# hzi-bifo/Quasimodo

Hardware: AMD Instinct MI355X
Metric: variant TP/FP classifications/sec across all caller x sample VCFs (higher is better)
Workload: dtype int32; 1 GPU; BASELINE configs[2]: 1000 VCFs x 1 M SNPs/GPU, 5 Mb ref, 100000 truth keys, 256-bin ROC, sorted; vcfs_per_gpu=1000, records_per_vcf=1000000, parallelism=vcf-shard x1, collective=none

## Files before the change

quasimodo_amd/csrc/qmvt_kernels.hip:

```cpp
#include <type_traits>
#include <hip/hip_runtime.h>
#include <stdint.h>
#include <stdlib.h>
#include <string.h>

#include "qmvt_dev.h"

namespace qm {

template <typename T> __device__ __forceinline__ T ntl(const T* p) {
  return __builtin_nontemporal_load(p);
}
template <typename T> __device__ __forceinline__ void nts(T* p, T v) {
  __builtin_nontemporal_store(v, p);
}
__device__ __forceinline__ int lane_id() { return (int)(threadIdx.x & 63); }
__device__ __forceinline__ uint64_t ballot64(bool p) { return __ballot(p); }
__device__ __forceinline__ int popc64(uint64_t x) { return __popcll(x); }

__device__ __forceinline__ int qual_bin(float q, int n_bins) {
  if (!(q >= 0.0f)) return -1;
  if (q >= (float)n_bins) return n_bins - 1;
  return (int)q;
}

__device__ __forceinline__ bool is_snp(int r, int a) { return ((uint32_t)r < 4u) & ((uint32_t)a < 4u); }
__device__ __forceinline__ uint32_t pack_key(int p, int r, int a) {
  return ((uint32_t)p << 4) | ((uint32_t)r << 2) | (uint32_t)a;
}

__device__ __forceinline__ int lds_lower_bound(const uint32_t* __restrict__ k, int m, int top, uint32_t key) {
  int pos = 0;
  for (int step = top; step > 0; step >>= 1) {
    int idx = pos + step;
    int rd = idx <= m ? idx - 1 : m - 1;
    uint32_t v = k[rd];
    if (idx <= m && v < key) pos = idx;
  }
  return pos;
}


constexpr uint32_t I_BIN1 = 0x1ffu;
constexpr uint32_t I_PASS = 1u << 9;
constexpr uint32_t I_IDDOT = 1u << 10;
constexpr uint32_t I_NOKEY = 1u << 11;
constexpr uint32_t I_LIVE = 1u << 12;
constexpr uint32_t I_BADPOS = 1u << 13;
constexpr uint32_t I_KEPT = 1u << 16;
constexpr uint32_t I_IDDOT4 = 1u << 20;
constexpr uint32_t I_TPLINE = 1u << 24;

__device__ __forceinline__ void pack_record_nib(int p, bool alive, uint32_t nib, float q, uint32_t fl, int nb, uint32_t& key, uint32_t& inf) {
  const bool okpos = (uint32_t)p < (uint32_t)QM_POS_LIMIT_DEV;
  const bool live = okpos && alive;
  key = ((uint32_t)p << 4) | (live ? nib : 0u);
  inf = (live ? (uint32_t)(qual_bin(q, nb) + 1) : 0u) | ((fl & 7u) << 9) | (live ? I_LIVE : 0u) | (okpos ? 0u : I_BADPOS) |
        ((live && (fl & QMF_PASS)) ? I_KEPT : 0u) | ((fl & QMF_IDDOT) ? I_IDDOT4 : 0u) | ((live && (fl & QMF_TPLINE)) ? I_TPLINE : 0u);
}
__device__ __forceinline__ void pack_record(int p, uint32_t d, float q, uint32_t fl, int nb, uint32_t& key, uint32_t& inf) {
  d &= 0xffu;
  pack_record_nib(p, d < 16u, d, q, fl, nb, key, inf);
}
__device__ __forceinline__ void pack_record_ext(int p, int r, int a, float q, uint32_t fl, int nb, uint32_t& key, uint32_t& inf) {
  pack_record_nib(p, allele_valid(r) && allele_valid(a), allele_nib(r, a), q, fl, nb, key, inf);
}

__host__ __device__ inline uint32_t flag_info(uint32_t f) {
  return ((f & 7u) << 9) | I_LIVE | ((f & QMF_PASS) ? I_KEPT : 0u) | ((f & QMF_IDDOT) ? I_IDDOT4 : 0u) | ((f & QMF_TPLINE) ? I_TPLINE : 0u);
}

__device__ __forceinline__ void pack_record_fast(int p, uint32_t d, float q, uint32_t f4x4 , float nbm1f,
                                                 const uint32_t* flut, uint32_t& key, uint32_t& inf) {
  const bool live = ((uint32_t)p | (d << 24)) < (uint32_t)QM_POS_LIMIT_DEV;
  key = ((uint32_t)p << 4) | (live ? d : 0u);
  const float c = fminf(fmaxf(q, -1.0f), nbm1f);
  const uint32_t b1 = (uint32_t)((int)floorf(c) + 1);
  const uint32_t g = *reinterpret_cast<const uint32_t*>(reinterpret_cast<const char*>(flut) + f4x4);
  inf = live ? (b1 | g) : 0u;
}

__device__ __forceinline__ void pack_record_fast_ext(int p, int r, int a, float q, uint32_t f4x4, float nbm1f, const uint32_t* flut,
                                                     uint32_t& key, uint32_t& inf) {
  const uint32_t ur = (uint32_t)r, ua = (uint32_t)a;
  constexpr uint32_t VALID_BY_CLZ = 0xC000001Eu;
  const uint32_t ok = (VALID_BY_CLZ >> __builtin_clz(ur | 1u)) & (VALID_BY_CLZ >> __builtin_clz(ua | 1u)) & 1u;
  const bool live = ((uint32_t)p >> 28) < ok;
  const uint32_t nib = ((ur << 2) ^ ua ^ ((ur ^ ua) >> 4)) & 15u;
  key = ((uint32_t)p << 4) | (live ? nib : 0u);
  const float c = fminf(fmaxf(q, -1.0f), nbm1f);
  const uint32_t b1 = (uint32_t)((int)floorf(c) + 1);
  const uint32_t g = *reinterpret_cast<const uint32_t*>(reinterpret_cast<const char*>(flut) + f4x4);
  inf = live ? (b1 | g) : 0u;
}

struct Cols {
  const int32_t* pos;
  const int32_t* ref;
  const int32_t* alt;
  const float* qual;
  const uint8_t* flags;
  const uint8_t* anib;
  const uint32_t* pkey;
  const uint32_t* pinf;
};

template <bool PACKED> struct Raw4;
template <> struct Raw4<false> { int4 p, r, a; float4 q; uint32_t f, d; };
template <> struct Raw4<true> { uint4 k, i; int4 r, a; };

template <bool EXT>
__device__ __forceinline__ void load_raw(const Cols& C, int idx, Raw4<false>& R) {
  typedef int v4i __attribute__((ext_vector_type(4)));
  typedef float v4f __attribute__((ext_vector_type(4)));
  const v4i vp = __builtin_nontemporal_load(reinterpret_cast<const v4i*>(C.pos + idx));
  if (EXT) {
    const v4i vr = __builtin_nontemporal_load(reinterpret_cast<const v4i*>(C.ref + idx));
    const v4i va = __builtin_nontemporal_load(reinterpret_cast<const v4i*>(C.alt + idx));
    R.r = make_int4(vr.x, vr.y, vr.z, vr.w);
    R.a = make_int4(va.x, va.y, va.z, va.w);
  } else {
    R.d = __builtin_nontemporal_load(reinterpret_cast<const uint32_t*>(C.anib + idx));
  }
  const v4f vq = __builtin_nontemporal_load(reinterpret_cast<const v4f*>(C.qual + idx));
  R.p = make_int4(vp.x, vp.y, vp.z, vp.w);
  R.q = make_float4(vq.x, vq.y, vq.z, vq.w);
  R.f = __builtin_nontemporal_load(reinterpret_cast<const uint32_t*>(C.flags + idx));
}
template <bool EXT>
__device__ __forceinline__ void load_raw(const Cols& C, int idx, Raw4<true>& R) {
  typedef unsigned v4u __attribute__((ext_vector_type(4)));
  const v4u vk = __builtin_nontemporal_load(reinterpret_cast<const v4u*>(C.pkey + idx));
  const v4u vi = __builtin_nontemporal_load(reinterpret_cast<const v4u*>(C.pinf + idx));
  R.k = make_uint4(vk.x, vk.y, vk.z, vk.w);
  R.i = make_uint4(vi.x, vi.y, vi.z, vi.w);
  if (EXT) {
    R.r = *reinterpret_cast<const int4*>(C.ref + idx);
    R.a = *reinterpret_cast<const int4*>(C.alt + idx);
  }
}

struct In4 {
  uint32_t key[4], inf[4];
  int32_t r[4], a[4];
  uint32_t posor;
};

template <bool EXT>
__device__ __forceinline__ void unpack_raw(const Raw4<false>& R, int nb, In4& X, const uint32_t* flut) {
  const float nbm1f = (float)(nb - 1);
  if (!EXT) {
    pack_record_fast(R.p.x, R.d & 0xffu, R.q.x, (R.f << 2) & 0x3cu, nbm1f, flut, X.key[0], X.inf[0]);
    pack_record_fast(R.p.y, (R.d >> 8) & 0xffu, R.q.y, (R.f >> 6) & 0x3cu, nbm1f, flut, X.key[1], X.inf[1]);
    pack_record_fast(R.p.z, (R.d >> 16) & 0xffu, R.q.z, (R.f >> 14) & 0x3cu, nbm1f, flut, X.key[2], X.inf[2]);
    pack_record_fast(R.p.w, R.d >> 24, R.q.w, (R.f >> 22) & 0x3cu, nbm1f, flut, X.key[3], X.inf[3]);
  } else {
    pack_record_fast_ext(R.p.x, R.r.x, R.a.x, R.q.x, (R.f << 2) & 0x3cu, nbm1f, flut, X.key[0], X.inf[0]);
    pack_record_fast_ext(R.p.y, R.r.y, R.a.y, R.q.y, (R.f >> 6) & 0x3cu, nbm1f, flut, X.key[1], X.inf[1]);
    pack_record_fast_ext(R.p.z, R.r.z, R.a.z, R.q.z, (R.f >> 14) & 0x3cu, nbm1f, flut, X.key[2], X.inf[2]);
    pack_record_fast_ext(R.p.w, R.r.w, R.a.w, R.q.w, (R.f >> 22) & 0x3cu, nbm1f, flut, X.key[3], X.inf[3]);
    X.r[0] = R.r.x; X.r[1] = R.r.y; X.r[2] = R.r.z; X.r[3] = R.r.w;
    X.a[0] = R.a.x; X.a[1] = R.a.y; X.a[2] = R.a.z; X.a[3] = R.a.w;
  }
  X.posor = (uint32_t)R.p.x | (uint32_t)R.p.y | (uint32_t)R.p.z | (uint32_t)R.p.w;
}
template <bool EXT>
__device__ __forceinline__ void unpack_raw(const Raw4<true>& R, int, In4& X, const uint32_t*) {
  X.posor = 0u;
  if (EXT) {
    X.r[0] = R.r.x; X.r[1] = R.r.y; X.r[2] = R.r.z; X.r[3] = R.r.w;
    X.a[0] = R.a.x; X.a[1] = R.a.y; X.a[2] = R.a.z; X.a[3] = R.a.w;
  }
  X.key[0] = R.k.x; X.key[1] = R.k.y; X.key[2] = R.k.z; X.key[3] = R.k.w;
  X.inf[0] = R.i.x; X.inf[1] = R.i.y; X.inf[2] = R.i.z; X.inf[3] = R.i.w;
}

typedef const __attribute__((address_space(4))) int32_t* ci32p;
typedef const __attribute__((address_space(4))) uint32_t* cu32p;
__device__ __forceinline__ int uload(const int32_t* p, int i) { return ((ci32p)(uintptr_t)p)[i]; }
__device__ __forceinline__ uint32_t uload(const uint32_t* p, int i) { return ((cu32p)(uintptr_t)p)[i]; }
template <bool PACKED> __device__ __forceinline__ int rec_pos_uniform(const Cols& C, int i) {
  if (PACKED) return (int)(uload(C.pkey, i) >> 4);
  return uload(C.pos, i);
}

template <bool PACKED> __device__ __forceinline__ int rec_pos(const Cols& C, int i) {
  if (PACKED) return (int)(C.pkey[i] >> 4);
  return C.pos[i];
}
template <bool PACKED, bool EXT = false>
__device__ __forceinline__ void rec_packed(const Cols& C, int i, int nb, uint32_t& key, uint32_t& inf) {
  if (PACKED) { key = C.pkey[i]; inf = C.pinf[i]; return; }
  if (EXT) pack_record_ext(C.pos[i], C.ref[i], C.alt[i], C.qual[i], C.flags[i], nb, key, inf);
  else pack_record(C.pos[i], C.anib[i], C.qual[i], C.flags[i], nb, key, inf);
}

typedef const __attribute__((address_space(1))) uint32_t* gu32p;
typedef const __attribute__((address_space(1))) int32_t* gi32p;
struct TruthG {
  gu32p keys;
  gi32p tidx;
  gi32p ref, alt;
  int32_t shift, nb;
};
template <bool EXT>
__device__ __forceinline__ TruthG truth_global(const TruthDev& t) {
  TruthG g;
  if (EXT) {
    g.keys = (gu32p)t.xkeys; g.tidx = (gi32p)t.xtidx; g.ref = (gi32p)t.xref; g.alt = (gi32p)t.xalt; g.shift = t.xshift; g.nb = t.xnb;
  } else {
    g.keys = (gu32p)t.keys; g.tidx = (gi32p)t.tidx; g.ref = nullptr; g.alt = nullptr; g.shift = t.shift; g.nb = t.nb;
  }
  return g;
}

constexpr int H_PACK = 1;
constexpr int L_HTP = 0;
constexpr int L_HFP = 130;
constexpr int L_HU = 260;
constexpr int L_KEYS = 388;
__device__ __forceinline__ void hist_add(uint32_t* lds, int table, uint32_t slot) {
  if (H_PACK) atomicAdd(&lds[table + (slot >> 1)], 1u << (16u * (slot & 1u)));
  else atomicAdd(&lds[table + slot], 1u);
}
__device__ __forceinline__ uint32_t hist_get(const uint32_t* lds, int table, uint32_t slot) {
  return H_PACK ? (lds[table + (slot >> 1)] >> (16u * (slot & 1u))) & 0xffffu : lds[table + slot];
}
constexpr int L_SMAX = L_KEYS + K1_SLICE;
constexpr int L_SRF = L_SMAX + K1_SLICE;
constexpr int L_RKEY = (L_SRF + K1_SLICE / 32 + 3) & ~3;
constexpr int L_RINF = L_RKEY + 288;
constexpr int L_HITS = L_RINF + 128;
constexpr int L_FLUT = L_HITS + 8;
constexpr int L_TCNT = L_FLUT + 16;
#ifndef QM_MASK_TILES
#define QM_MASK_TILES 8
#endif
#ifndef QM_MASK_TILES_X
#define QM_MASK_TILES_X 4
#endif

template <bool EXT> __device__ __forceinline__ constexpr int mask_tiles() { return EXT ? QM_MASK_TILES_X : QM_MASK_TILES; }
constexpr int L_MASK = (L_TCNT + 2 * SPAN_TILES + 3) & ~3;
constexpr int L_TOTAL = L_MASK + 64 * QM_MASK_TILES;
constexpr int L_XRREF = L_MASK + 64 * QM_MASK_TILES_X;
constexpr int L_XRALT = L_XRREF + 256;
constexpr int L_TOTAL_X = L_XRALT + 256;
constexpr int SLICE_CAP_X = K1_SLICE / 2;
template <bool EXT> __device__ __forceinline__ constexpr int slice_cap() { return EXT ? SLICE_CAP_X : K1_SLICE; }
static_assert(L_XRREF % 4 == 0, "b128 LDS stores need natural alignment");
static_assert(L_RKEY % 4 == 0 && L_RINF % 2 == 0, "b128 / b64 LDS stores need natural alignment");
static_assert(K1_ROUNDS == 4, "a tile is 32 + 32 mask words");
static_assert(SPAN_TILES % QM_MASK_TILES == 0 && SPAN_TILES % QM_MASK_TILES_X == 0 && (32 * QM_MASK_TILES) % 8 == 0, "mask batches tile the span");
static_assert(K1_ROUNDS >= 3 && K1_SLICE % 64 == 0, "the next tile's slice is fetched over rounds 0..2 of the current one");

__device__ __forceinline__ int rk(int i) { return L_RKEY + i + ((i >> 5) << 2); }

struct Slice {
  int keys, smax, srf;
  int ref, alt;
  int m;
};

__device__ __forceinline__ void slice_select(Slice& S) {
  S.keys = L_KEYS;
  S.smax = L_SMAX;
  S.srf = L_SRF;
  S.ref = L_KEYS + SLICE_CAP_X;
  S.alt = L_SMAX + SLICE_CAP_X;
}

template <bool EXT>
__device__ __forceinline__ void stage_slice(uint32_t* lds, const TruthG& tr, int c0, const Slice& S, int lane) {
  for (int j = lane; j < S.m; j += 64) {
    lds[S.keys + j] = tr.keys[c0 + j];
    lds[S.smax + j] = 0;
    if (EXT) { lds[S.ref + j] = (uint32_t)tr.ref[c0 + j]; lds[S.alt + j] = (uint32_t)tr.alt[c0 + j]; }
  }
  if (lane < K1_SLICE / 32) lds[S.srf + lane] = 0;
}

__device__ __forceinline__ void slice_range(const TruthG& tr, int a, int b, int& lo, int& hi) {
  uint32_t ba = (uint32_t)a >> tr.shift;
  uint32_t bb = ((uint32_t)b >> tr.shift) + 1u;
  const uint32_t lim = (uint32_t)tr.nb + 1u;
  ba = ba < lim ? ba : lim;
  bb = bb < lim ? bb : lim;
  lo = uload((const int32_t*)(uintptr_t)tr.tidx, (int)ba);
  hi = uload((const int32_t*)(uintptr_t)tr.tidx, (int)bb);
  if (hi < lo) hi = lo;
}

struct SegBounds {
  int a, b;
  int prevp, nextp;
};

template <bool PACKED> __device__ __forceinline__ SegBounds seg_bounds(const Cols& C, int sb, int se, int vn) {
  SegBounds t;
  t.a = rec_pos_uniform<PACKED>(C, sb);
  t.b = rec_pos_uniform<PACKED>(C, se - 1);
  t.prevp = (sb > 0) ? rec_pos_uniform<PACKED>(C, sb - 1) : INT32_MIN;
  t.nextp = (se < vn) ? rec_pos_uniform<PACKED>(C, se) : INT32_MIN;
  return t;
}

template <bool EXT>
__device__ __forceinline__ void stage_round(uint32_t* lds, In4& X, int i0, int te, int lane) {
  if (i0 - lane * 4 + 256 > te) {
#pragma unroll
    for (int k = 0; k < 4; ++k)
      if (i0 + k >= te) { X.key[k] = 0xffffffffu; X.inf[k] = 0u; }
  }
  uint4 kv;
  kv.x = X.key[0]; kv.y = X.key[1]; kv.z = X.key[2]; kv.w = X.key[3];
  uint2 iv;
  iv.x = (X.inf[0] & 0xffffu) | (X.inf[1] << 16); iv.y = (X.inf[2] & 0xffffu) | (X.inf[3] << 16);
  *reinterpret_cast<uint4*>(&lds[rk(lane * 4)]) = kv;
  *reinterpret_cast<uint2*>(&lds[L_RINF + lane * 2]) = iv;
  if (EXT) {
    uint4 rv, av;
    rv.x = (uint32_t)X.r[0]; rv.y = (uint32_t)X.r[1]; rv.z = (uint32_t)X.r[2]; rv.w = (uint32_t)X.r[3];
    av.x = (uint32_t)X.a[0]; av.y = (uint32_t)X.a[1]; av.z = (uint32_t)X.a[2]; av.w = (uint32_t)X.a[3];
    *reinterpret_cast<uint4*>(&lds[L_XRREF + lane * 4]) = rv;
    *reinterpret_cast<uint4*>(&lds[L_XRALT + lane * 4]) = av;
  }
  if (lane < 8) lds[L_HITS + lane] = 0;
}

template <bool EXT>
__device__ __forceinline__ void join_round(uint32_t* lds, const Slice& S, int nrec, int own_a, int lane) {
  if (S.m <= 0 || nrec <= 0) return;
  const uint32_t first_pos = lds[rk(0)] >> 4;
  const uint32_t last_pos = lds[rk(nrec - 1)] >> 4;
  int rlo = 0, rhi = 0;
  for (int base = 0; base < S.m; base += 64) {
    const int j = base + lane;
    const uint32_t kp = j < S.m ? lds[S.keys + j] >> 4 : 0xffffffffu;
    rlo += popc64(ballot64(kp < first_pos));
    rhi += popc64(ballot64(kp <= last_pos));
  }
  for (int base = rlo; base < rhi; base += 64) {
    const int j = base + lane;
    if (j < rhi) {
      const uint32_t kkey = lds[S.keys + j];
      const uint32_t kpos = kkey >> 4;
      const uint32_t kfloor = kkey & ~15u;
      int pp = 0;
#pragma unroll
      for (int st = 144; st >= 36; st >>= 1)
        if (lds[L_RKEY + pp + st - 5] < kfloor) pp += st;
#pragma unroll
      for (int st = 16; st > 0; st >>= 1)
        if (lds[L_RKEY + pp + st - 1] < kfloor) pp += st;
      int s = pp - 4 * ((pp * 1821) >> 16);
      if (s < 256 && lds[L_RKEY + pp] < kfloor) s += 1;
      uint32_t mx = 0, rf = 0;
      for (; s < nrec; ++s) {
        const uint32_t rkey = lds[rk(s)];
        if ((rkey & ~15u) != kfloor) break;
        if (rkey != kkey) continue;
        if (EXT) {
          if (lds[L_XRREF + s] != lds[S.ref + j] || lds[L_XRALT + s] != lds[S.alt + j]) continue;
        }
        const uint32_t inf = (lds[L_RINF + (s >> 1)] >> (16 * (s & 1))) & 0xffffu;
        if ((inf & (I_LIVE | I_NOKEY)) != I_LIVE) continue;
        atomicOr(&lds[L_HITS + (s >> 5)], 1u << (s & 31));
        if ((int)kpos != own_a) {
          const uint32_t b1 = inf & I_BIN1;
          if ((inf & I_IDDOT) && b1 > mx) mx = b1;
          rf |= (inf & I_PASS) ? 1u : 0u;
        }
      }
      if (mx) atomicMax(&lds[S.smax + j], mx);
      if (rf) atomicOr(&lds[S.srf + (j >> 5)], 1u << (j & 31));
    }
  }
}

__device__ __forceinline__ int slice_lower_bound(const uint32_t* lds, const Slice& S, uint32_t key) {
  int lo = 0, n = S.m;
  while (n > 0) {
    const int h = n >> 1;
    if (lds[S.keys + lo + h] < key) { lo += h + 1; n -= h + 1; } else n = h;
  }
  return lo;
}

template <bool PACKED, bool EXT>
__device__ __forceinline__ void continue_run(const Cols& C, uint32_t* lds, const Slice& S, int se, int vn, int bpos, int nb, int lane) {
  for (int base = se; base < vn; base += 64) {
    const int i = base + lane;
    bool cont = false;
    if (i < vn) {
      cont = (rec_pos<PACKED>(C, i) == bpos);
      if (cont && S.m > 0) {
        uint32_t key, inf;
        rec_packed<PACKED, EXT>(C, i, nb, key, inf);
        if ((inf & (I_LIVE | I_NOKEY)) == I_LIVE) {
          int j = slice_lower_bound(lds, S, key);
          if (EXT) {
            const uint32_t rr = (uint32_t)C.ref[i], aa = (uint32_t)C.alt[i];
            while (j < S.m && lds[S.keys + j] == key && (lds[S.ref + j] != rr || lds[S.alt + j] != aa)) ++j;
          }
          if (j < S.m && lds[S.keys + j] == key) {
            if (inf & I_IDDOT) atomicMax(&lds[S.smax + j], inf & I_BIN1);
            if (inf & I_PASS) atomicOr(&lds[S.srf + (j >> 5)], 1u << (j & 31));
          }
        }
      }
    }
    if (ballot64(cont) != ~0ull) break;
  }
}

__device__ __forceinline__ uint32_t flush_slice(uint32_t* lds, const Slice& S, int lane) {
  uint32_t tpr = 0;
  for (int j = lane; j < S.m; j += 64) {
    const uint32_t mx = lds[S.smax + j];
    if (mx) hist_add(lds, L_HU, mx - 1u);
    tpr += (lds[S.srf + (j >> 5)] >> (j & 31)) & 1u;
  }
  return tpr;
}

constexpr int X_WALK_LIMIT = 1 << 14;
template <bool PACKED, bool EXT>
__device__ __forceinline__ uint32_t repeated_key(const Cols& C, int i, uint32_t key, uint32_t nokey, int nb, int32_t r, int32_t a,
                                                 uint32_t& bad) {
  for (int j = i - 1; j >= 0; --j) {
    if (EXT && i - j > X_WALK_LIMIT) { bad |= 4u; break; }
    if (rec_pos<PACKED>(C, j) != (int)(key >> 4)) break;
    uint32_t kj, ij;
    rec_packed<PACKED, EXT>(C, j, nb, kj, ij);
    if (kj == key && (ij & (I_LIVE | I_PASS)) == (I_LIVE | I_PASS) && (ij & I_NOKEY) == nokey) {
      if (!EXT || (C.ref[j] == r && C.alt[j] == a)) return 1u;
    }
  }
  return 0u;
}

struct Acc {
  uint32_t bad;
  uint32_t fpr;
  uint32_t n_pass, n_tp;
  uint32_t top_tp, top_fp;
  uint32_t posor;
};

__device__ __forceinline__ uint32_t or_reduce8(uint32_t v) {
  v |= (uint32_t)__builtin_amdgcn_update_dpp(0, (int)v, 0x111, 0xf, 0xf, false);
  v |= (uint32_t)__builtin_amdgcn_update_dpp(0, (int)v, 0x112, 0xf, 0xf, false);
  v |= (uint32_t)__builtin_amdgcn_update_dpp(0, (int)v, 0x114, 0xf, 0xf, false);
  return v;
}

template <bool PACKED, bool EXT>
__device__ __forceinline__ void classify_round(uint32_t* lds, const Cols& C, const In4& X, int rbase, int te, int prev_last, int nb,
                                               int mslot, Acc& A, int lane) {
  const uint32_t hit = (lds[L_HITS + (lane >> 3)] >> (4 * (lane & 7))) & 15u;
  uint32_t nib = 0, anyinf = 0;
#pragma unroll
  for (int k = 0; k < 4; ++k) {
    nib |= (X.inf[k] >> 16) << k;
    anyinf |= X.inf[k];
  }
  const uint32_t pass = nib & 15u, iddot = (nib >> 4) & 15u, tpline = (nib >> 8) & 15u;
  A.bad |= ((anyinf & I_BADPOS) | (X.posor >> 28)) ? 2u : 0u;
  A.posor |= X.posor;
  const uint32_t tpkey = (hit & iddot) | tpline;
  const uint32_t tp = pass & tpkey;
  const uint32_t fpkey = pass & ~hit;
  A.n_pass += (uint32_t)__popc(pass);
  A.n_tp += (uint32_t)__popc(tp);
  A.fpr += (uint32_t)__popc(fpkey);
  {
    const uint32_t sh = 4u * (uint32_t)(lane & 7);
    const uint32_t wp = or_reduce8(pass << sh);
    const uint32_t wt = or_reduce8(tp << sh);
    if ((lane & 7) == 7) {
      lds[L_MASK + mslot + (lane >> 3)] = wp;
      lds[L_MASK + 32 * mask_tiles<EXT>() + mslot + (lane >> 3)] = wt;
    }
  }
  int pp = __shfl_up((int)(X.key[3] >> 4), 1);
  if (lane == 0) pp = prev_last;
  const int i0 = rbase + lane * 4;
  uint32_t cand = 0;
#pragma unroll
  for (int k = 0; k < 4; ++k) {
    const int p = (int)(X.key[k] >> 4);
    A.bad |= (p < pp) ? 1u : 0u;
    cand |= ((p == pp) ? 1u : 0u) << k;
    {
      const uint32_t b1 = X.inf[k] & I_BIN1;
      const uint32_t notp = ((~tpkey) >> k) & 1u;
      const bool top = b1 == (uint32_t)nb;
      const uint64_t mtop = ballot64(top);
      if (mtop) {
        const uint32_t ntp = (uint32_t)popc64(ballot64(top && !notp));
        A.top_tp += ntp;
        A.top_fp += (uint32_t)popc64(mtop) - ntp;
      }
      if (!top) hist_add(lds, notp ? L_HFP : L_HTP, b1);
    }
    pp = p;
  }
  cand &= fpkey;
  if (cand) {
#pragma unroll
    for (int k = 0; k < 4; ++k)
      if ((cand >> k) & 1u) {
        const int32_t rr = EXT ? (int32_t)lds[L_XRREF + lane * 4 + k] : 0, aa = EXT ? (int32_t)lds[L_XRALT + lane * 4 + k] : 0;
        A.fpr -= repeated_key<PACKED, EXT>(C, i0 + k, X.key[k], X.inf[k] & I_NOKEY, nb, rr, aa, A.bad);
      }
  }
}

__device__ __forceinline__ uint32_t wave_sum(uint32_t v) {
#define QM_DPP_ADD(ctrl, rmask) v += (uint32_t)__builtin_amdgcn_update_dpp(0, (int)v, ctrl, rmask, 0xf, false)
  QM_DPP_ADD(0xb1, 0xf);
  QM_DPP_ADD(0x4e, 0xf);
  QM_DPP_ADD(0x141, 0xf);
  QM_DPP_ADD(0x140, 0xf);
  QM_DPP_ADD(0x142, 0xa);
  QM_DPP_ADD(0x143, 0xc);
#undef QM_DPP_ADD
  return (uint32_t)__builtin_amdgcn_readlane((int)v, 63);
}

#ifndef K1_WAVES_PER_EU
#define K1_WAVES_PER_EU 5
#endif
#ifndef K1_WAVES_EXT_MIN
#define K1_WAVES_EXT_MIN 5
#endif
#ifndef K1_WAVES_MAX
#define K1_WAVES_MAX 5
#endif

template <bool PACKED, bool EXT>
__global__ __launch_bounds__(64) __attribute__((amdgpu_waves_per_eu(EXT ? K1_WAVES_EXT_MIN : K1_WAVES_PER_EU, K1_WAVES_MAX))) void k_classify(ClassifyParams P) {
  __shared__ __attribute__((aligned(16))) uint32_t lds[(EXT ? L_TOTAL_X : L_TOTAL)];

  const int lane = (int)threadIdx.x;
  const int bid_ = (int)blockIdx.x;
  const int span_id = bid_ + P.span_base;
  const SpanDesc sp = P.spans[span_id];
  const TruthG tr = truth_global<EXT>(P.truths[sp.truth]);
  Cols C;
  C.pos = P.pos + sp.voff; C.ref = P.ref + sp.voff; C.alt = P.alt + sp.voff; C.qual = P.qual + sp.voff; C.flags = P.flags + sp.voff;
  C.anib = P.anib + sp.voff;
  C.pkey = P.pkey + sp.voff; C.pinf = P.pinf + sp.voff;
  uint32_t* const mpass32 = reinterpret_cast<uint32_t*>(P.mask_pass + (sp.voff >> 6));
  uint32_t* const mtp32 = reinterpret_cast<uint32_t*>(P.mask_tp + (sp.voff >> 6));
  const int vn = sp.vn;
  const int sp_end = (int)(sp.end - sp.voff);
  const int nb = P.n_bins;

  for (int i = lane; i < L_KEYS; i += 64) lds[i] = 0;
  if (lane < 16) lds[L_FLUT + lane] = flag_info((uint32_t)lane);
  if (P.zero_acc && blockIdx.x == 0)
    for (int i = lane; i < P.zero_words; i += 64) P.zero_acc[i] = 0ull;
  if (!PACKED && P.known && P.known[sp.vcf]) return;
  Acc A = {0u, 0u, 0u, 0u, 0u, 0u, 0u};
  uint32_t acc_pass = 0, acc_tp = 0;
  uint32_t acc_tpr = 0;

  int tb = (int)(sp.begin - sp.voff);
  int te = (tb + K1_TILE < sp_end) ? tb + K1_TILE : sp_end;
  Raw4<PACKED> N;
  load_raw<EXT>(C, tb + lane * 4, N);
  int spos = 0;
  if constexpr (!PACKED) if (vn >= 4096) spos = C.pos[(int)(((int64_t)lane * vn) >> 6)];
  SegBounds B = seg_bounds<PACKED>(C, tb, te, vn);
  if constexpr (!PACKED) {
    const int n0 = te - tb < 256 ? te - tb : 256;
    const int j = lane * 4;
    const int pl = __shfl_up(N.p.w, 1);
    const bool ooo = (j + 1 < n0 && N.p.y < N.p.x) || (j + 2 < n0 && N.p.z < N.p.y) || (j + 3 < n0 && N.p.w < N.p.z) || (lane > 0 && j < n0 && N.p.x < pl);
    uint32_t po = (j < n0 ? (uint32_t)N.p.x : 0u) | (j + 1 < n0 ? (uint32_t)N.p.y : 0u) | (j + 2 < n0 ? (uint32_t)N.p.z : 0u) | (j + 3 < n0 ? (uint32_t)N.p.w : 0u);
    const int spl = __shfl_up(spos, 1);
    const bool sooo = vn >= 4096 && lane > 0 && spos < spl;
    po |= vn >= 4096 ? (uint32_t)spos : 0u;
    if (ballot64(ooo || sooo) != 0ull && ballot64((po >> 28) != 0u) == 0ull) {
      for (int o = 32; o > 0; o >>= 1) po |= (uint32_t)__shfl_xor((int)po, o);
      if (lane < 8) P.span_scal[(size_t)span_id * 8 + lane] = lane == 5 ? (uint32_t)SPANF_UNSORTED : lane == 6 ? po : 0u;
      return;
    }
  }
  int lo, hi;
  slice_range(tr, B.a, B.b, lo, hi);
  Slice S;
  slice_select(S);
  S.m = (hi - lo) <= slice_cap<EXT>() ? (hi - lo) : 0;
  stage_slice<EXT>(lds, tr, lo, S, lane);
  __syncthreads();

  int tile = sp.tile0;
  for (;;) {
    const bool has_next_tile = te < sp_end;
    const int ntb = tb + K1_TILE;
    const int nte = (ntb + K1_TILE < sp_end) ? ntb + K1_TILE : sp_end;
    const bool oversize = (hi - lo) > slice_cap<EXT>();
    const bool started_before = (tb > 0) && (B.prevp == B.a);
    const int own_a = started_before ? B.a : INT32_MIN;
    const bool owns_b = !(started_before && B.a == B.b);
    const int nrounds = (te - tb + 255) >> 8;

    SegBounds NB = B;
    int nlo = 0, nhi = 0;
    constexpr int NSL = (EXT ? SLICE_CAP_X : K1_SLICE) / 64;
    uint32_t nkeys[NSL], nref[NSL], nalt[NSL];
#pragma unroll
    for (int q = 0; q < NSL; ++q) { nkeys[q] = 0u; nref[q] = 0u; nalt[q] = 0u; }
    int prev_last = B.prevp;
    for (int r = 0; r < nrounds; ++r) {
      In4 X;
      unpack_raw<EXT>(N, nb, X, lds + L_FLUT);
      const int rbase = tb + r * 256;
      const int rend = rbase + 256 < te ? rbase + 256 : te;
      if (has_next_tile) {
        if (r == 0) {
          NB = seg_bounds<PACKED>(C, ntb, nte, vn);
        } else if (r == 1) {
          slice_range(tr, NB.a, NB.b, nlo, nhi);
        } else if (r == 2) {
          const int nm = (nhi - nlo) <= slice_cap<EXT>() ? (nhi - nlo) : 0;
#pragma unroll
          for (int q = 0; q < NSL; ++q) {
            const bool in = q * 64 + lane < nm;
            nkeys[q] = in ? tr.keys[nlo + q * 64 + lane] : 0u;
            if (EXT) { nref[q] = in ? (uint32_t)tr.ref[nlo + q * 64 + lane] : 0u; nalt[q] = in ? (uint32_t)tr.alt[nlo + q * 64 + lane] : 0u; }
          }
        }
      }
      if (rbase + 256 < sp_end) load_raw<EXT>(C, rbase + 256 + lane * 4, N);
      stage_round<EXT>(lds, X, rbase + lane * 4, te, lane);
      __syncthreads();
      {
        if (!oversize) {
          join_round<EXT>(lds, S, rend - rbase, own_a, lane);
        } else {
          const int pl = __shfl_up((int)(X.key[3] >> 4), 1);
          const bool ooo = (lane > 0 && X.key[0] != 0xffffffffu && (int)(X.key[0] >> 4) < pl) ||
                           (X.key[1] < (X.key[0] & ~15u)) || (X.key[2] < (X.key[1] & ~15u)) || (X.key[3] < (X.key[2] & ~15u));
          if (ballot64(ooo) != 0ull) {
            A.bad |= 1u;
          } else {
            const SegBounds RB = seg_bounds<PACKED>(C, rbase, rend, vn);
            const bool r_started = (rbase > 0) && (RB.prevp == RB.a);
            const int r_own_a = r_started ? RB.a : INT32_MIN;
            int rlo, rhi;
            slice_range(tr, RB.a, RB.b, rlo, rhi);
            for (int c0 = rlo; c0 < rhi; c0 += slice_cap<EXT>()) {
              S.m = (rhi - c0) < slice_cap<EXT>() ? (rhi - c0) : slice_cap<EXT>();
              stage_slice<EXT>(lds, tr, c0, S, lane);
              __syncthreads();
              join_round<EXT>(lds, S, rend - rbase, r_own_a, lane);
              if (RB.nextp == RB.b && !(r_started && RB.a == RB.b)) continue_run<PACKED, EXT>(C, lds, S, rend, vn, RB.b, nb, lane);
              __syncthreads();
              acc_tpr += flush_slice(lds, S, lane);
              __syncthreads();
            }
            S.m = 0;
          }
        }
      }
      __syncthreads();
      classify_round<PACKED, EXT>(lds, C, X, rbase, te, prev_last, nb, 32 * ((tile - sp.tile0) % mask_tiles<EXT>()) + 8 * r, A, lane);
      prev_last = (int)(lds[rk(255)] >> 4);
      __syncthreads();
    }

    if (!oversize) {
      if (B.nextp == B.b && owns_b) continue_run<PACKED, EXT>(C, lds, S, te, vn, B.b, nb, lane);
      __syncthreads();
      acc_tpr += flush_slice(lds, S, lane);
    }
    {
      const uint32_t tile_np = wave_sum(A.n_pass), tile_nt = wave_sum(A.n_tp);
      A.n_pass = 0; A.n_tp = 0;
      if (lane == 0) {
        lds[L_TCNT + (tile - sp.tile0)] = tile_nt;
        lds[L_TCNT + SPAN_TILES + (tile - sp.tile0)] = tile_np - tile_nt;
      }
      acc_pass += tile_np;
      acc_tp += tile_nt;
    }
    const bool stop_unsorted = !PACKED && ballot64(A.bad & 1u) != 0ull;
    {
      constexpr int MT = mask_tiles<EXT>();
      const int tin = (tile - sp.tile0) % MT;
      if (tin == MT - 1 || !has_next_tile || stop_unsorted) {
        __syncthreads();
        const int b0 = tb - tin * K1_TILE;
        const int nd = ((te - b0 + 255) >> 8) * 8;
#pragma unroll
        for (int half = 0; half < 2; ++half) {
          uint32_t* dst = (half ? mtp32 : mpass32) + (b0 >> 5);
          const int src = L_MASK + half * 32 * MT;
          for (int w = 4 * lane; w < 32 * MT; w += 256) {
            constexpr bool mask_nt = true;
            if (w + 3 < nd) {
              typedef unsigned v4u_ __attribute__((ext_vector_type(4)));
              if (mask_nt) __builtin_nontemporal_store(*reinterpret_cast<const v4u_*>(&lds[src + w]), reinterpret_cast<v4u_*>(dst + w));
              else *reinterpret_cast<uint4*>(dst + w) = *reinterpret_cast<const uint4*>(&lds[src + w]);
            }
            else for (int k = 0; k < 4; ++k) if (w + k < nd) dst[w + k] = lds[src + w + k];
          }
        }
      }
    }

    if (!has_next_tile) break;
    if (stop_unsorted) break;
    B = NB;
    tb = ntb;
    te = nte;
    ++tile;
    lo = nlo;
    hi = nhi;
    S.m = (hi - lo) <= slice_cap<EXT>() ? (hi - lo) : 0;
#pragma unroll
    for (int q = 0; q < NSL; ++q) {
      const int j = q * 64 + lane;
      if (j < S.m) {
        lds[S.keys + j] = nkeys[q]; lds[S.smax + j] = 0;
        if (EXT) { lds[S.ref + j] = nref[q]; lds[S.alt + j] = nalt[q]; }
      }
    }
    if (lane < K1_SLICE / 32) lds[S.srf + lane] = 0;
    __syncthreads();
  }

  acc_tpr = wave_sum(acc_tpr);
  A.fpr = wave_sum(A.fpr);
  const uint64_t any_uns = ballot64(A.bad & 1u);
  const uint64_t any_bad = ballot64(A.bad & 2u);
  const uint64_t any_lim = ballot64(A.bad & 4u);
  __syncthreads();
  const uint32_t top_tp = A.top_tp, top_fp = A.top_fp;
  uint32_t* oh = P.span_hist + (size_t)span_id * SPAN_HIST_WORDS;
  for (int i = lane; i < 128; i += 64) {
    const int b0 = 2 * i, b1 = 2 * i + 1;
#define K1_HST(p, x) (*(p) = (x))
    K1_HST(&oh[i], (hist_get(lds, L_HTP, 1 + b0) + (b0 == nb - 1 ? top_tp : 0u)) | ((hist_get(lds, L_HTP, 1 + b1) + (b1 == nb - 1 ? top_tp : 0u)) << 16));
    K1_HST(&oh[128 + i], (hist_get(lds, L_HFP, 1 + b0) + (b0 == nb - 1 ? top_fp : 0u)) | ((hist_get(lds, L_HFP, 1 + b1) + (b1 == nb - 1 ? top_fp : 0u)) << 16));
    K1_HST(&oh[256 + i], hist_get(lds, L_HU, b0) | (hist_get(lds, L_HU, b1) << 16));
#undef K1_HST
  }
  {
    const int nt_span = (sp_end - (int)(sp.begin - sp.voff) + K1_TILE - 1) / K1_TILE;
    const int t = lane & (SPAN_TILES - 1);
    if (lane < 2 * SPAN_TILES && t < nt_span) (lane < SPAN_TILES ? P.tile_tp : P.tile_fp)[sp.tile0 + t] = lds[L_TCNT + lane];
  }
  if (lane == 0) {
    uint32_t* sc = P.span_scal + (size_t)span_id * 8;
    sc[0] = acc_pass; sc[1] = acc_tp; sc[2] = acc_pass - acc_tp; sc[3] = acc_tpr; sc[4] = A.fpr;
    sc[5] = (any_uns ? SPANF_UNSORTED : 0u) | (any_bad ? SPANF_BADPOS : 0u) | (any_lim ? SPANF_RUNLIMIT : 0u);
    sc[7] = 0;
  }
  {
    uint32_t po = A.posor;
    for (int o = 32; o > 0; o >>= 1) po |= (uint32_t)__shfl_xor((int)po, o);
    if (lane == 0) P.span_scal[(size_t)span_id * 8 + 6] = po;
  }
}

__global__ __launch_bounds__(256) void k_finalize(FinalizeParams P) {
  __shared__ uint32_t s_h[3][4];
  __shared__ uint32_t s_scan[256];
  const int v = (int)blockIdx.x + P.vcf_base;
  const int tid = (int)threadIdx.x;
  const VcfDesc vd = P.vcfs[v];
  const int row_cap = P.row_cap ? ((int)P.row_cap[v] > 1 ? (int)P.row_cap[v] : 1) : HB_BUCKETS;
  const int nb = P.n_bins;

  __shared__ unsigned long long s_sc[5];
  __shared__ uint32_t s_fl, s_or;
  if (tid < 5) s_sc[tid] = 0ull;
  if (tid == 5) s_fl = 0u;
  if (tid == 6) s_or = 0u;
  __syncthreads();
  for (int i = tid; i < vd.nspans * 8; i += 256) {
    if (P.row_cap && ((i >> 3) & (HB_BUCKETS - 1)) >= row_cap) continue;
    const uint32_t x = P.span_scal[(size_t)vd.span0 * 8 + i];
    const int k = i & 7;
    if (k < 5) { if (x) atomicAdd(&s_sc[k], (unsigned long long)x); }
    else if (k == 5) { if (x) atomicOr(&s_fl, x); }
    else if (k == 6) { if (x) atomicOr(&s_or, x); }
  }
  const bool rows = (P.parts & 2) != 0, offsets = (P.parts & 1) != 0;
  auto write_flags = [&](uint32_t fl) {
    if (P.vcf_posor) P.vcf_posor[v] = s_or;
    const uint32_t out = fl & (SPANF_UNSORTED | SPANF_BADPOS | SPANF_RUNLIMIT | SPANF_OVERFLOW);
    P.vcf_flags[v] = out;
    if (P.host_flags) {
      __hip_atomic_store(P.host_flags + v, out, __ATOMIC_RELAXED, __HIP_MEMORY_SCOPE_SYSTEM);
      __hip_atomic_store(P.host_aux + v, P.row_cap ? P.row_cap[v] : s_or, __ATOMIC_RELAXED, __HIP_MEMORY_SCOPE_SYSTEM);
    }
    if (P.chunk_bad && ((out & (SPANF_OVERFLOW | SPANF_BADPOS)) || (P.row_cap && P.row_cap[v] > P.row_cap_limit))) atomicOr(P.chunk_bad, 1u);
  };
  if (P.lazy_unsorted) {
    __syncthreads();
    if (s_fl & SPANF_UNSORTED) {
      if (offsets && tid == 5) write_flags(s_fl);
      return;
    }
  }
  __shared__ uint32_t s_part[2][4][256];
  uint32_t h0 = 0, h1 = 0, h2 = 0, hsub = 0;
  if (rows) {
    const int w = tid & 127, g = tid >> 7;
    uint32_t a0 = 0, a1 = 0, b0 = 0, b1 = 0, c0 = 0, c1 = 0, u0 = 0, u1 = 0;
#pragma unroll 8
    for (int s = g; s < vd.nspans; s += 2) {
      if (P.row_cap && (s & (HB_BUCKETS - 1)) >= row_cap) continue;
      const uint32_t* sh = P.span_hist + (size_t)(vd.span0 + s) * SPAN_HIST_WORDS;
      const uint32_t x = sh[w], y = sh[128 + w], z = sh[256 + w];
      a0 += x & 0xffffu; a1 += x >> 16; b0 += y & 0xffffu; b1 += y >> 16; c0 += z & 0xffffu; c1 += z >> 16;
      if (s < HB_BUCKETS) { u0 += x & 0xffffu; u1 += x >> 16; }
    }
    s_part[g][0][2 * w] = a0; s_part[g][0][2 * w + 1] = a1; s_part[g][1][2 * w] = b0; s_part[g][1][2 * w + 1] = b1;
    s_part[g][2][2 * w] = c0; s_part[g][2][2 * w + 1] = c1; s_part[g][3][2 * w] = u0; s_part[g][3][2 * w + 1] = u1;
  }
  __syncthreads();
  if (rows) {
    h0 = s_part[0][0][tid] + s_part[1][0][tid]; h1 = s_part[0][1][tid] + s_part[1][1][tid];
    h2 = s_part[0][2][tid] + s_part[1][2][tid]; hsub = s_part[0][3][tid] + s_part[1][3][tid];
    if (P.all_hist && tid < nb) h1 += P.all_hist[(size_t)v * SEG_HIST_WORDS + 1 + tid] - hsub;
  }
  {
    const int lane = tid & 63, wave = tid >> 6;
    uint32_t i0 = h0, i1 = h1, i2 = h2;
#pragma unroll
    for (int o = 1; o < 64; o <<= 1) {
      const uint32_t y0 = __shfl_down(i0, o), y1 = __shfl_down(i1, o), y2 = __shfl_down(i2, o);
      if (lane + o < 64) { i0 += y0; i1 += y1; i2 += y2; }
    }
    if (lane == 0) { s_h[0][wave] = i0; s_h[1][wave] = i1; s_h[2][wave] = i2; }
    __syncthreads();
    uint64_t c0 = i0, c1 = i1, c2 = i2;
    for (int w = wave + 1; w < 4; ++w) { c0 += s_h[0][w]; c1 += s_h[1][w]; c2 += s_h[2][w]; }
    const uint32_t fl = s_fl;
    const bool unsorted = (fl & SPANF_UNSORTED) != 0u;
    if (rows && tid < nb) {
      uint64_t* roc = P.roc + (size_t)v * 3 * nb;
      roc[tid] = c0; roc[nb + tid] = c1; roc[2 * nb + tid] = c2;
      if (P.global_acc && !unsorted) {
        unsigned long long* g = reinterpret_cast<unsigned long long*>(P.global_acc) + (size_t)vd.truth * 3 * nb;
        if (c0) atomicAdd(&g[tid], (unsigned long long)c0);
        if (c1) atomicAdd(&g[nb + tid], (unsigned long long)c1);
        if (c2) atomicAdd(&g[2 * nb + tid], (unsigned long long)c2);
      }
    }
    if (rows && tid < 8) {
      int64_t* sc = P.scalars + (size_t)v * 8;
      if (tid < 5) sc[tid] = (int64_t)s_sc[tid];
      else if (tid == 5) sc[5] = unsorted ? 0 : 1;
      else if (tid == 6) sc[6] = vd.n;
      else sc[7] = P.ext ? P.truths[vd.truth].xn : P.truths[vd.truth].n;
    }
    if (offsets && tid == 5) write_flags(fl);
  }
  if (!offsets) return;
  {
    const int lane = tid & 63, wave = tid >> 6;
    uint32_t fsum = 0;
    for (int i = tid; i < vd.ntiles; i += 256) fsum += P.tile_fp[vd.tile0 + i];
    fsum = wave_sum(fsum);
    if (lane == 0) s_scan[8 + wave] = fsum;
    __syncthreads();
    const uint32_t fp_total = s_scan[8] + s_scan[9] + s_scan[10] + s_scan[11];
    uint32_t carry_t = 0, carry_f = (uint32_t)vd.n - fp_total;
    if (tid == 0 && P.vcf_tot) P.vcf_tot[2 * v + 1] = fp_total;
    for (int base = 0; base < vd.ntiles; base += 1024) {
      const int t0 = base + tid * 4;
      uint32_t xt[4], xf[4];
#pragma unroll
      for (int k = 0; k < 4; ++k) {
        const bool in = t0 + k < vd.ntiles;
        xt[k] = in ? P.tile_tp[vd.tile0 + t0 + k] : 0u;
        xf[k] = in ? P.tile_fp[vd.tile0 + t0 + k] : 0u;
      }
      const uint32_t st = xt[0] + xt[1] + xt[2] + xt[3], sf = xf[0] + xf[1] + xf[2] + xf[3];
      uint32_t it = st, jf = sf;
#pragma unroll
      for (int o = 1; o < 64; o <<= 1) {
        const uint32_t yt = __shfl_up(it, o), yf = __shfl_up(jf, o);
        if (lane >= o) { it += yt; jf += yf; }
      }
      if (lane == 63) { s_scan[wave] = it; s_scan[4 + wave] = jf; }
      __syncthreads();
      uint32_t wt = 0, wf = 0, bt = 0, bf = 0;
#pragma unroll
      for (int w = 0; w < 4; ++w) {
        const uint32_t a = s_scan[w], c = s_scan[4 + w];
        wt += w < wave ? a : 0u; wf += w < wave ? c : 0u;
        bt += a; bf += c;
      }
      uint32_t et = carry_t + wt + it - st, ef = carry_f + wf + jf - sf;
#pragma unroll
      for (int k = 0; k < 4; ++k) {
        if (t0 + k < vd.ntiles) { P.tile_tp_off[vd.tile0 + t0 + k] = et; P.tile_fp_off[vd.tile0 + t0 + k] = ef; }
        et += xt[k]; ef += xf[k];
      }
      carry_t += bt; carry_f += bf;
      __syncthreads();
    }
    if (tid == 0 && P.vcf_tot) P.vcf_tot[2 * v] = carry_t;
  }
}

#ifndef K3_TILES
#define K3_TILES 4
#endif
#ifndef K3_WAVES
#define K3_WAVES 4
#endif
static_assert(SPAN_TILES % (K3_WAVES * K3_TILES) == 0, "a workgroup's tiles lie in one span");
constexpr int K3_PASS = 512;
static_assert(K1_TILE == 2 * K3_PASS, "a tile is two passes");
constexpr int K3_NPASS = 2 * K3_TILES;
#ifndef K3_FCH_LOG
#define K3_FCH_LOG 8
#endif
#ifndef K3_TCH_LOG
#define K3_TCH_LOG 6
#endif
static_assert(K3_FCH_LOG >= 4 && K3_FCH_LOG <= 8 && K3_TCH_LOG >= 4 && K3_TCH_LOG <= 8, "a chunk is whole 64-byte pieces, at most one store instruction");
constexpr int K3_EXTRA = 2;
static_assert(K3_EXTRA * K3_PASS == K1_TILE, "a wave reaches exactly one tile beyond its own");
constexpr int K3_BUF = 256 + K3_PASS + 16;

struct K3Lut {
  uint32_t w[512];
  constexpr K3Lut() : w() {
    for (int v = 0; v < 256; ++v) {
      uint64_t l = 0;
      int n = 0;
      for (int b = 0; b < 8; ++b)
        if ((v >> b) & 1) { l |= (uint64_t)b << (8 * n); ++n; }
      w[2 * v] = (uint32_t)l;
      w[2 * v + 1] = (uint32_t)(l >> 32);
    }
  }
};
__device__ const K3Lut k3_lut = K3Lut();

typedef volatile uint32_t __attribute__((address_space(3)))* k3_ldsp;
typedef int k3_v4i __attribute__((ext_vector_type(4)));
typedef volatile k3_v4i __attribute__((address_space(3)))* k3_lds4p;

template <int K> __device__ __forceinline__ uint32_t k3_or_byte(uint32_t base, uint32_t l) {
  uint32_t r;
  if (K == 0) asm("v_or_b32_sdwa %0, %1, %2 dst_sel:DWORD dst_unused:UNUSED_PAD src0_sel:BYTE_0 src1_sel:DWORD" : "=v"(r) : "v"(l), "v"(base));
  if (K == 1) asm("v_or_b32_sdwa %0, %1, %2 dst_sel:DWORD dst_unused:UNUSED_PAD src0_sel:BYTE_1 src1_sel:DWORD" : "=v"(r) : "v"(l), "v"(base));
  if (K == 2) asm("v_or_b32_sdwa %0, %1, %2 dst_sel:DWORD dst_unused:UNUSED_PAD src0_sel:BYTE_2 src1_sel:DWORD" : "=v"(r) : "v"(l), "v"(base));
  if (K == 3) asm("v_or_b32_sdwa %0, %1, %2 dst_sel:DWORD dst_unused:UNUSED_PAD src0_sel:BYTE_3 src1_sel:DWORD" : "=v"(r) : "v"(l), "v"(base));
  return r;
}
__device__ __forceinline__ void k3_emit(k3_ldsp buf, const uint32_t* lut, uint32_t a, uint32_t m, uint32_t base) {
  if (m) {
    const uint2 l = *reinterpret_cast<const uint2*>(&lut[2 * m]);
    k3_ldsp d = buf + a;
    d[7] = k3_or_byte<3>(base, l.y);
    d[6] = k3_or_byte<2>(base, l.y);
    d[5] = k3_or_byte<1>(base, l.y);
    d[4] = k3_or_byte<0>(base, l.y);
    d[3] = k3_or_byte<3>(base, l.x);
    d[2] = k3_or_byte<2>(base, l.x);
    d[1] = k3_or_byte<1>(base, l.x);
    d[0] = k3_or_byte<0>(base, l.x);
  }
}
__device__ __forceinline__ uint32_t k3_scan(uint32_t c, uint32_t& tot) {
  uint32_t x = c;
#define K3_DPP_ADD(ctrl, rmask) x += (uint32_t)__builtin_amdgcn_update_dpp(0, (int)x, ctrl, rmask, 0xf, false)
  K3_DPP_ADD(0x111, 0xf);
  K3_DPP_ADD(0x112, 0xf);
  K3_DPP_ADD(0x114, 0xf);
  K3_DPP_ADD(0x118, 0xf);
  K3_DPP_ADD(0x142, 0xa);
  K3_DPP_ADD(0x143, 0xc);
#undef K3_DPP_ADD
  tot = (uint32_t)__builtin_amdgcn_readlane((int)x, 63);
  return x;
}

struct K3List {
  k3_ldsp buf;
  int32_t* out;
  uint32_t lo, hi;
  uint32_t g0;
  uint32_t n;
};
__device__ __forceinline__ void k3_store4(int32_t* p, k3_v4i w) {
  __builtin_nontemporal_store(w, reinterpret_cast<k3_v4i*>(p));
}
__device__ __forceinline__ void k3_store_part(const K3List& X, uint32_t c0, uint32_t lo, uint32_t hi, int lane) {
  const uint32_t b = X.g0 + c0;
  const uint32_t q = b + 4u * (uint32_t)lane;
  if (q >= lo && q + 4u <= hi) k3_store4(X.out + q, *reinterpret_cast<k3_lds4p>(X.buf + (c0 + 4u * lane)));
  if (lane < 6) {
    const uint32_t lo4 = (lo + 3u) & ~3u, hi4 = hi & ~3u;
    uint32_t i = lane < 3 ? lo + (uint32_t)lane : hi4 + (uint32_t)(lane - 3);
    const bool ok = lane < 3 ? (i < lo4 && i < hi) : (i < hi && i >= lo && i >= lo4);
    if (ok) X.out[i] = (int32_t)X.buf[i - X.g0];
  }
}
template <int CL>
__device__ __forceinline__ void k3_drain(K3List& X, int lane) {
  const uint32_t nfull = X.n >> CL;
  if (!nfull) return;
  const uint32_t top = X.g0 + (nfull << CL);
  const uint32_t s0 = X.lo > X.g0 ? X.lo : X.g0, e0 = X.hi < top ? X.hi : top;
  for (uint32_t w = X.g0; w < e0; w += 256u) {
    if (w + 256u <= s0) continue;
    if (s0 <= w && w + 256u <= e0) k3_store4(X.out + w + 4u * lane, *reinterpret_cast<k3_lds4p>(X.buf + ((w - X.g0) + 4u * lane)));
    else k3_store_part(X, w - X.g0, s0 > w ? s0 : w, e0 < w + 256u ? e0 : w + 256u, lane);
  }
  const uint32_t left = X.n - (nfull << CL);
  if (4u * (uint32_t)lane < left) {
    const k3_v4i v = *reinterpret_cast<k3_lds4p>(X.buf + ((nfull << CL) + 4u * lane));
    *reinterpret_cast<k3_lds4p>(X.buf + 4u * lane) = v;
  }
  X.g0 = top;
  X.n = left;
}
template <int CL>
__device__ __forceinline__ void k3_own(K3List& X, uint32_t a, uint32_t a2, uint32_t aprev, uint32_t rnext, uint32_t reach, uint32_t l0, uint32_t l1) {
  constexpr uint32_t M = (1u << CL) - 1u, C = 1u << CL;
  const uint32_t s = a & ~M;
  const uint32_t up = (a + M) & ~M, up2 = (a2 + M) & ~M;
  const bool head = a == l0;
  const bool begins = up < a2 || (head && a2 > a);
  const uint32_t sb = s > l0 ? s : l0;
  const bool inherited = !head && s != a && sb >= aprev && sb < a;
  X.lo = inherited ? (s + C < rnext ? s + C : rnext) : a;
  const uint32_t end = up2 < reach ? up2 : reach;
  X.hi = begins ? (end < l1 ? end : l1) : a2;
  X.g0 = s;
  X.n = a - s;
}

__global__ __launch_bounds__(64 * K3_WAVES) void k_compact(CompactParams P) {
  __shared__ __attribute__((aligned(16))) uint32_t s_buf[K3_WAVES][2][K3_BUF];
  __shared__ __attribute__((aligned(16))) uint32_t s_lut[512];
  const int tid = (int)threadIdx.x, lane = tid & 63;
  const int wave = __builtin_amdgcn_readfirstlane(tid >> 6);
// ... 1986 lines not shown
```

Measured before the change: 301.7 billion classifications/s.

## Micro-optimize record packing, ROC histogram layout, and incremental truth-slice join window

Several independent tweaks to the per-tile classify kernel. Quality binning now uses a med3 clamp with a floor-convert instruction, and info packing uses add and byte-permute instead of masks and shifts. The TP and FP histograms are merged into one interleaved table, so each record does a single LDS atomic whose increment is chosen arithmetically rather than by branching between tables. The join window scan now resumes from the previous round's lower bound and stops early once keys pass the round's last position, cutting repeated ballot scans over the truth slice. The carried window and the packed 16-bit counters assume sorted input and per-span counts below 65536.

```diff
diff --git a/quasimodo_amd/csrc/qmvt_kernels.hip b/quasimodo_amd/csrc/qmvt_kernels.hip
--- a/quasimodo_amd/csrc/qmvt_kernels.hip
+++ b/quasimodo_amd/csrc/qmvt_kernels.hip
@@ -70,14 +70,20 @@
   return ((f & 7u) << 9) | I_LIVE | ((f & QMF_PASS) ? I_KEPT : 0u) | ((f & QMF_IDDOT) ? I_IDDOT4 : 0u) | ((f & QMF_TPLINE) ? I_TPLINE : 0u);
 }
 
+__device__ __forceinline__ uint32_t qual_bin1_fast(float q, float nbm1f) {
+  const float c = __builtin_amdgcn_fmed3f(__builtin_canonicalizef(q), -1.0f, nbm1f);
+  int b;
+  asm("v_cvt_flr_i32_f32 %0, %1" : "=v"(b) : "v"(c));
+  return (uint32_t)(b + 1);
+}
+
 __device__ __forceinline__ void pack_record_fast(int p, uint32_t d, float q, uint32_t f4x4 , float nbm1f,
                                                  const uint32_t* flut, uint32_t& key, uint32_t& inf) {
   const bool live = ((uint32_t)p | (d << 24)) < (uint32_t)QM_POS_LIMIT_DEV;
   key = ((uint32_t)p << 4) | (live ? d : 0u);
-  const float c = fminf(fmaxf(q, -1.0f), nbm1f);
-  const uint32_t b1 = (uint32_t)((int)floorf(c) + 1);
+  const uint32_t b1 = qual_bin1_fast(q, nbm1f);
   const uint32_t g = *reinterpret_cast<const uint32_t*>(reinterpret_cast<const char*>(flut) + f4x4);
-  inf = live ? (b1 | g) : 0u;
+  inf = live ? (b1 + g) : 0u;
 }
 
 __device__ __forceinline__ void pack_record_fast_ext(int p, int r, int a, float q, uint32_t f4x4, float nbm1f, const uint32_t* flut,
@@ -88,10 +94,9 @@
   const bool live = ((uint32_t)p >> 28) < ok;
   const uint32_t nib = ((ur << 2) ^ ua ^ ((ur ^ ua) >> 4)) & 15u;
   key = ((uint32_t)p << 4) | (live ? nib : 0u);
-  const float c = fminf(fmaxf(q, -1.0f), nbm1f);
-  const uint32_t b1 = (uint32_t)((int)floorf(c) + 1);
+  const uint32_t b1 = qual_bin1_fast(q, nbm1f);
   const uint32_t g = *reinterpret_cast<const uint32_t*>(reinterpret_cast<const char*>(flut) + f4x4);
-  inf = live ? (b1 | g) : 0u;
+  inf = live ? (b1 + g) : 0u;
 }
 
 struct Cols {
@@ -147,8 +152,7 @@
 };
 
 template <bool EXT>
-__device__ __forceinline__ void unpack_raw(const Raw4<false>& R, int nb, In4& X, const uint32_t* flut) {
-  const float nbm1f = (float)(nb - 1);
+__device__ __forceinline__ void unpack_raw(const Raw4<false>& R, float nbm1f, In4& X, const uint32_t* flut) {
   if (!EXT) {
     pack_record_fast(R.p.x, R.d & 0xffu, R.q.x, (R.f << 2) & 0x3cu, nbm1f, flut, X.key[0], X.inf[0]);
     pack_record_fast(R.p.y, (R.d >> 8) & 0xffu, R.q.y, (R.f >> 6) & 0x3cu, nbm1f, flut, X.key[1], X.inf[1]);
@@ -165,7 +169,7 @@
   X.posor = (uint32_t)R.p.x | (uint32_t)R.p.y | (uint32_t)R.p.z | (uint32_t)R.p.w;
 }
 template <bool EXT>
-__device__ __forceinline__ void unpack_raw(const Raw4<true>& R, int, In4& X, const uint32_t*) {
+__device__ __forceinline__ void unpack_raw(const Raw4<true>& R, float, In4& X, const uint32_t*) {
   X.posor = 0u;
   if (EXT) {
     X.r[0] = R.r.x; X.r[1] = R.r.y; X.r[2] = R.r.z; X.r[3] = R.r.w;
@@ -215,8 +219,7 @@
 }
 
 constexpr int H_PACK = 1;
-constexpr int L_HTP = 0;
-constexpr int L_HFP = 130;
+constexpr int L_HROC = 0;
 constexpr int L_HU = 260;
 constexpr int L_KEYS = 388;
 __device__ __forceinline__ void hist_add(uint32_t* lds, int table, uint32_t slot) {
@@ -315,7 +318,8 @@
   uint4 kv;
   kv.x = X.key[0]; kv.y = X.key[1]; kv.z = X.key[2]; kv.w = X.key[3];
   uint2 iv;
-  iv.x = (X.inf[0] & 0xffffu) | (X.inf[1] << 16); iv.y = (X.inf[2] & 0xffffu) | (X.inf[3] << 16);
+  iv.x = __builtin_amdgcn_perm(X.inf[1], X.inf[0], 0x05040100u);
+  iv.y = __builtin_amdgcn_perm(X.inf[3], X.inf[2], 0x05040100u);
   *reinterpret_cast<uint4*>(&lds[rk(lane * 4)]) = kv;
   *reinterpret_cast<uint2*>(&lds[L_RINF + lane * 2]) = iv;
   if (EXT) {
@@ -329,17 +333,20 @@
 }
 
 template <bool EXT>
-__device__ __forceinline__ void join_round(uint32_t* lds, const Slice& S, int nrec, int own_a, int lane) {
+__device__ __forceinline__ void join_round(uint32_t* lds, const Slice& S, int nrec, int own_a, int lane, int& wlo) {
   if (S.m <= 0 || nrec <= 0) return;
   const uint32_t first_pos = lds[rk(0)] >> 4;
   const uint32_t last_pos = lds[rk(nrec - 1)] >> 4;
-  int rlo = 0, rhi = 0;
-  for (int base = 0; base < S.m; base += 64) {
+  int rlo = wlo, rhi = wlo;
+  for (int base = wlo; base < S.m; base += 64) {
     const int j = base + lane;
     const uint32_t kp = j < S.m ? lds[S.keys + j] >> 4 : 0xffffffffu;
+    const int nh = popc64(ballot64(kp <= last_pos));
     rlo += popc64(ballot64(kp < first_pos));
-    rhi += popc64(ballot64(kp <= last_pos));
-  }
+    rhi += nh;
+    if (nh < 64) break;
+  }
+  wlo = rlo;
   for (int base = rlo; base < rhi; base += 64) {
     const int j = base + lane;
     if (j < rhi) {
@@ -495,14 +502,14 @@
     {
       const uint32_t b1 = X.inf[k] & I_BIN1;
       const uint32_t notp = ((~tpkey) >> k) & 1u;
-      const bool top = b1 == (uint32_t)nb;
-      const uint64_t mtop = ballot64(top);
+      const bool below = b1 != (uint32_t)nb;
+      const uint64_t mtop = ~ballot64(below);
       if (mtop) {
-        const uint32_t ntp = (uint32_t)popc64(ballot64(top && !notp));
+        const uint32_t ntp = (uint32_t)popc64(mtop & ~ballot64(notp != 0u));
         A.top_tp += ntp;
         A.top_fp += (uint32_t)popc64(mtop) - ntp;
       }
-      if (!top) hist_add(lds, notp ? L_HFP : L_HTP, b1);
+      if (below) atomicAdd(&lds[L_HROC + b1], notp * 0xffffu + 1u);
     }
     pp = p;
   }
@@ -557,6 +564,7 @@
   const int vn = sp.vn;
   const int sp_end = (int)(sp.end - sp.voff);
   const int nb = P.n_bins;
+  const float nbm1f = (float)(nb - 1);
 
   for (int i = lane; i < L_KEYS; i += 64) lds[i] = 0;
   if (lane < 16) lds[L_FLUT + lane] = flag_info((uint32_t)lane);
@@ -615,9 +623,10 @@
 #pragma unroll
     for (int q = 0; q < NSL; ++q) { nkeys[q] = 0u; nref[q] = 0u; nalt[q] = 0u; }
     int prev_last = B.prevp;
+    int wlo = 0;
     for (int r = 0; r < nrounds; ++r) {
       In4 X;
-      unpack_raw<EXT>(N, nb, X, lds + L_FLUT);
+      unpack_raw<EXT>(N, nbm1f, X, lds + L_FLUT);
       const int rbase = tb + r * 256;
       const int rend = rbase + 256 < te ? rbase + 256 : te;
       if (has_next_tile) {
@@ -640,7 +649,7 @@
       __syncthreads();
       {
         if (!oversize) {
-          join_round<EXT>(lds, S, rend - rbase, own_a, lane);
+          join_round<EXT>(lds, S, rend - rbase, own_a, lane, wlo);
         } else {
           const int pl = __shfl_up((int)(X.key[3] >> 4), 1);
           const bool ooo = (lane > 0 && X.key[0] != 0xffffffffu && (int)(X.key[0] >> 4) < pl) ||
@@ -657,7 +666,8 @@
               S.m = (rhi - c0) < slice_cap<EXT>() ? (rhi - c0) : slice_cap<EXT>();
               stage_slice<EXT>(lds, tr, c0, S, lane);
               __syncthreads();
-              join_round<EXT>(lds, S, rend - rbase, r_own_a, lane);
+              int w0 = 0;
+              join_round<EXT>(lds, S, rend - rbase, r_own_a, lane, w0);
               if (RB.nextp == RB.b && !(r_started && RB.a == RB.b)) continue_run<PACKED, EXT>(C, lds, S, rend, vn, RB.b, nb, lane);
               __syncthreads();
               acc_tpr += flush_slice(lds, S, lane);
@@ -745,8 +755,8 @@
   for (int i = lane; i < 128; i += 64) {
     const int b0 = 2 * i, b1 = 2 * i + 1;
 #define K1_HST(p, x) (*(p) = (x))
-    K1_HST(&oh[i], (hist_get(lds, L_HTP, 1 + b0) + (b0 == nb - 1 ? top_tp : 0u)) | ((hist_get(lds, L_HTP, 1 + b1) + (b1 == nb - 1 ? top_tp : 0u)) << 16));
-    K1_HST(&oh[128 + i], (hist_get(lds, L_HFP, 1 + b0) + (b0 == nb - 1 ? top_fp : 0u)) | ((hist_get(lds, L_HFP, 1 + b1) + (b1 == nb - 1 ? top_fp : 0u)) << 16));
+    K1_HST(&oh[i], ((lds[L_HROC + 1 + b0] & 0xffffu) + (b0 == nb - 1 ? top_tp : 0u)) | (((lds[L_HROC + 1 + b1] & 0xffffu) + (b1 == nb - 1 ? top_tp : 0u)) << 16));
+    K1_HST(&oh[128 + i], ((lds[L_HROC + 1 + b0] >> 16) + (b0 == nb - 1 ? top_fp : 0u)) | (((lds[L_HROC + 1 + b1] >> 16) + (b1 == nb - 1 ? top_fp : 0u)) << 16));
     K1_HST(&oh[256 + i], hist_get(lds, L_HU, b0) | (hist_get(lds, L_HU, b1) << 16));
 #undef K1_HST
   }
```

Result: faster. 320.3 billion classifications/s, median of 6 (+6.2%).
